# lmb-freiburg/locov

Hardware: AMD Instinct MI355X
Metric: proposals/sec through LSM ROI-head (1333x800, 1000 prop, 1203-class text bank) (higher is better)
Workload: dtype f32 (Res5 GEMM products formed from f16x2 split operands on the f16 matrix pipe, f32 accumulate; error vs f64 <= 1.5 x the f32-MFMA kernel's + 6e-7 and <= 3e-6 on every tested shape, tests/test_gpu_split_gemm.py)

## Files before the change

include/locov_hip.h:

```cpp
#ifndef LOCOV_HIP_H
#define LOCOV_HIP_H

#include <stdint.h>

#ifdef __cplusplus
extern "C" {
#endif

#define LOCOV_ABI_VERSION 8

#define LOCOV_OK 0
#define LOCOV_ERR_INVALID_ARG (-1)
#define LOCOV_ERR_LAUNCH (-2)
#define LOCOV_ERR_UNSUPPORTED (-3)

#define LOCOV_F32 0
#define LOCOV_BF16 1

#define LOCOV_NORM_NONE 0
#define LOCOV_NORM_L2 1
#define LOCOV_NORM_STANDARDIZE 2

#define LOCOV_EPI_RELU 1u
#define LOCOV_GEMM_A_SPLIT 0x1000u
// ... 428 lines not shown
} locov_weight_prep_job;
int locov_res5_weight_prep(const locov_weight_prep_job *jobs, int n_jobs, unsigned *overflow, locov_stream_t stream);

int locov_weight_transpose_scale(const float *w, int N, int K, const float *row_scale, float *out,
                                 locov_stream_t stream);
int locov_conv3x3_weight_flip(const float *w, int N, int Cin, const float *row_scale, float *out,
                              locov_stream_t stream);
int locov_im2col3x3_nhwc(const float *x, int64_t R, int H, int W, int C, float *col, locov_stream_t stream);
int locov_conv3x3_wgrad_unpack(const float *dw_packed, int N, int Cin, const float *row_scale, float *dw,
                               locov_stream_t stream);
int locov_relu_mask(const float *g, const float *act, int64_t n, float *out, float *amax_out, locov_stream_t stream);
#define LOCOV_ZERO_LIST_MAX 24
int locov_zero_if_raised(float *const *tensors, const int64_t *counts, int n_tensors, const unsigned *flag,
                         locov_stream_t stream);

int locov_spatial_mean_bwd(const float *g, const float *act, int64_t R, int C, int HW, float *out,
                           float *amax_out, locov_stream_t stream);
int locov_rows_stride2(const float *src, int N, int H, int W, int C, int forward, float *dst,
                       locov_stream_t stream);
int locov_roi_align_nhwc_bwd(const float *grad_rows, int64_t grad_ld, int N, int H, int W, int C,
                             const float *rois, int64_t R, int pooled_h, int pooled_w, float spatial_scale,
                             int sampling_ratio, int aligned, int bin_stride, int pos_major, float *grad_feat,
                             locov_stream_t stream);

#define LOCOV_REGIONS_MAX_B 64
#define LOCOV_REGIONS_MAX_CANDIDATES 4096
#define LOCOV_REGIONS_GRID 0
#define LOCOV_REGIONS_GRID_ALL 1
#define LOCOV_REGIONS_BOXES 2
#define LOCOV_REGIONS_ROWS 0
#define LOCOV_REGIONS_NCHW 1
int locov_regions_select(const double *keys, int mode, int B, const int *count_host, const int *ext_a_host,
                         const int *ext_b_host, int grid_w, const float *const *boxes_host, int n, int limit, int mask_w,
                         int mvm_w, int64_t *indices, int *src_row, int *inv, uint8_t *mask, float *loc, float *mvm,
                         locov_stream_t stream);
int locov_regions_gather_fwd(const float *src, int layout, int64_t ld, int B, int n, int C, int64_t hw, const int *src_row,
                             float *out, locov_stream_t stream);
int locov_regions_gather_bwd(const float *grad_out, int layout, int64_t ld, int64_t rows, int C, int64_t hw, const int *inv,
                             float *grad_src, locov_stream_t stream);

#define LOCOV_MHA_MAX_S 4096
#define LOCOV_MHA_MAX_GRID 65535
int locov_mha_fwd(const float *q, int64_t ldq, const float *k, int64_t ldk, const float *v, int64_t ldv, const float *bias,
                  const uint8_t *keep, float p_drop, float scale, int nseq, int S, int H, int d, float *ctx, int64_t ldo,
                  float *lse, locov_stream_t stream);
int locov_mha_bwd(const float *q, int64_t ldq, const float *k, int64_t ldk, const float *v, int64_t ldv, const float *bias,
// ... 68 lines not shown
```

locov_amd/_lib.py:

```python
from __future__ import annotations

import ctypes
import os
from ctypes import c_char_p, c_double, c_float,c_int, c_int64, c_uint, c_void_p, POINTER

HERE = os.path.dirname(os.path.abspath(__file__))
LIB_PATH = os.environ.get("LOCOV_HIP_LIB") or os.path.join(HERE, "liblocov_hip.so")

OK = 0
F32, BF16 = 0, 1
NORM_NONE, NORM_L2, NORM_STANDARDIZE = 0, 1, 2
EPI_RELU = 1
WINO_OUT_ROI_MAJOR = 0x100
WINO_IN_ROI_MAJOR = 0x200
SEGMEAN_RES_ROI_MAJOR = 0x400
GEMM_A_SPLIT = 0x1000
EPI_OUT_SPLIT = 0x2000
EPI_RES_SPLIT = 0x4000
MAX_LEVELS = 8
ZERO_LIST_MAX = 24
LABEL_MAX_IMAGES, LABEL_MAX_THRESHOLDS, SAMPLE_MAX_PROPOSALS = 64, 6, 4096
ABI_VERSION = 8
DETECT_MAX_CANDIDATES, DETECT_FLAG_NONFINITE, DETECT_FLAG_OVERFLOW = 8192, 1, 2
RPN_FLAG_NONFINITE, RPN_MAX_PRE_NMS_TOPK, RPN_MAX_ANCHORS = 1, 16384, (1 << 22) - 1
# ... 157 lines not shown
    "locov_winograd_wgrad_f32_split": (c_int, [_p, _p, c_int64, c_int, c_int, c_uint, _p, _p, _p, _p, c_int64, _p]),
    "locov_winograd_wgrad_f32_split_v": (c_int, [_p, _p, c_int64, c_int, c_int, c_uint, _p, _p, _p, _p, c_int64, _p]),
    "locov_conv1x1_winograd_workspace_bytes": (c_int64, [c_int64, c_int, c_int]),
    "locov_conv1x1_winograd_workspace_bytes_for": (c_int64, [c_int64, c_int, c_int, c_int, c_int64]),
    "locov_roi_align_winograd_workspace_bytes": (c_int64, [c_int64, c_int, c_int]),
    "locov_roi_align_winograd_conv3x3_f32_split": (c_int, [_p, c_int, c_int, c_int, c_int, c_int64, _p, c_int64, c_int, c_float, c_int, c_int,
                                                           _p, _p, _p, c_float, c_float, _p, _p, _p, c_int64, c_int, c_uint, c_float, _p, c_int64,
                                                           _p, _p]),
    "locov_conv1x1_winograd_conv3x3_f32_split": (c_int, [_p, c_int64, c_int, c_float, _p, c_float, _p, _p, c_int64, c_int, _p, c_float, c_float,
                                                         _p, _p, _p, c_int64, c_int, c_uint, c_float, _p, c_int64, _p, _p]),
    "locov_winograd_wgrad_workspace_bytes": (c_int64, [c_int64, c_int, c_int]),
    "locov_winograd_wgrad_f32": (c_int, [_p, _p, c_int64, c_int, c_int, c_uint, _p, _p, _p, c_int64, _p]),
    "locov_res5_weight_prep": (c_int, [POINTER(WeightPrepJob), c_int, _p, _p]),
    "locov_weight_transpose_scale": (c_int, [_p, c_int, c_int, _p, _p, _p]),
    "locov_conv3x3_weight_flip": (c_int, [_p, c_int, c_int, _p, _p, _p]),
    "locov_im2col3x3_nhwc": (c_int, [_p, c_int64, c_int, c_int, c_int, _p, _p]),
    "locov_conv3x3_wgrad_unpack": (c_int, [_p, c_int, c_int, _p, _p, _p]),
    "locov_relu_mask": (c_int, [_p, _p, c_int64, _p, _p, _p]),
    "locov_zero_if_raised": (c_int, [POINTER(c_void_p), POINTER(c_int64), c_int, _p, _p]),
    "locov_spatial_mean_bwd": (c_int, [_p, _p, c_int64, c_int, c_int, _p, _p, _p]),
    "locov_rows_stride2": (c_int, [_p, c_int, c_int, c_int, c_int, c_int, _p, _p]),
    "locov_roi_align_nhwc_bwd": (c_int, [_p, c_int64, c_int, c_int, c_int, c_int, _p, c_int64, c_int, c_int, c_float, c_int, c_int,
                                         c_int, c_int, _p, _p]),
    "locov_box_head_fwd": (c_int, [_p, c_int64, c_int, c_int, c_int, _p, _p, _p, _p, _p, _p, c_int, c_int,
                                   c_int, c_int, _p, _p, _p, _p, _p, _p]),
    "locov_regions_select": (c_int, [_p, c_int, c_int, POINTER(c_int), POINTER(c_int), POINTER(c_int), c_int, POINTER(c_void_p), c_int, c_int,
                                     c_int, c_int, _p, _p, _p, _p, _p, _p, _p]),
    "locov_regions_gather_fwd": (c_int, [_p, c_int, c_int64, c_int, c_int, c_int, c_int64, _p, _p, _p]),
    "locov_regions_gather_bwd": (c_int, [_p, c_int, c_int64, c_int64, c_int, c_int64, _p, _p, _p]),
    "locov_mha_fwd": (c_int, [_p, c_int64, _p, c_int64, _p, c_int64, _p, _p, c_float, c_float, c_int, c_int, c_int, c_int, _p, c_int64,
                              _p, _p]),
    "locov_mha_bwd": (c_int, [_p, c_int64, _p, c_int64, _p, c_int64, _p, _p, c_float, c_float, c_int, c_int, c_int, c_int, _p,
                              c_int64, _p, _p, _p, c_int64, _p, c_int64, _p, c_int64, _p]),
    "locov_resnet_stem_fwd": (c_int, [_p, c_int, c_int, c_int, _p, _p, _p, c_int, _p, _p]),
    "locov_resnet_stem_fwd_sel": (c_int, [_p, c_int, c_int, c_int, _p, _p, _p, c_int, _p, _p, _p]),
    "locov_resnet_stem_wgrad_workspace_bytes": (c_int64, [c_int, c_int, c_int]),
    "locov_resnet_stem_wgrad": (c_int, [_p, c_int, c_int, c_int, _p, _p, _p, c_int, _p, _p, c_int64, _p]),
    "locov_preprocess_images": (c_int, [POINTER(c_void_p), POINTER(c_int), POINTER(c_int), c_int, c_int, c_int, POINTER(c_float),
                                        POINTER(c_float), c_float, _p, c_int, c_int, _p]),
    "locov_detector_rescale": (c_int, [_p, POINTER(c_int), POINTER(c_float), POINTER(c_float), POINTER(c_int), POINTER(c_int), c_int,
                                       _p, _p, _p, _p]),
    "locov_caption_embed_fwd": (c_int, [_p, _p, c_int, c_int, c_int, c_int, _p, _p, c_int, _p, c_int, _p, _p, c_float, _p, c_float, c_double,
                                        c_double, c_double, c_int, c_int, c_int, _p, _p, _p, _p, _p, _p]),
    "locov_caption_embed_bwd_workspace_bytes": (c_int64, [c_int, c_int, c_int]),
    "locov_caption_embed_bwd": (c_int, [_p, c_int, c_int, c_int, c_int, _p, _p, _p, _p, _p, _p, _p, c_float, _p, _p, _p, _p, c_int64, _p]),
    "locov_sgd_workspace_bytes": (c_int64, [c_int, c_int64]),
# ... 43 lines not shown
```

locov_amd/csrc/roi_align_nhwc_bwd.hip:

```cpp
#include "roi_align_nhwc_common.h"

#include <cstdlib>

namespace locov {

__global__ __launch_bounds__(kNhwcThreads) void roi_align_nhwc_bwd_kernel(
    const float *__restrict__ grad_rows, int64_t grad_ld, float *__restrict__ grad_feat, int N, int H, int W, int C,
    const float *__restrict__ rois, int PH, int PW, float scale, int sampling_ratio, int aligned, int bin_stride, int OH, int OW,
    int pos_major, int nslices, int64_t R, int bwd_win_floats)
{
    extern __shared__ float bwd_win[];
    __shared__ AxisSampleN ytab[kMaxAxisN];
    __shared__ AxisSampleN xtab[kMaxAxisN];
    __shared__ float ypw[kSepCols * (kSepGrid + 1)];
    __shared__ float xpw[kSepCols * (kSepGrid + 1)];
    __shared__ int ypix[kSepCols][2];
    __shared__ int xpix[kSepCols][2];
    __shared__ int sep_bad;
    const NhwcRoiFrame f = nhwc_roi_frame(rois, N, H, W, C, PH, PW, scale, sampling_ratio, aligned, bin_stride, OH, OW, (int64_t)C,
                                          (unsigned)sizeof(float), nslices, R, NhwcRoiLds{ytab, xtab, ypw, xpw, ypix, xpix, &sep_bad});
    const float start_h = f.start_h, start_w = f.start_w, bin_h = f.bin_h, bin_w = f.bin_w, inv_count = f.inv_count;
    const int gh = f.gh, gw = f.gw, q_lo = f.q_lo;
    const unsigned xstride = f.xstride, ystride = f.ystride;
    const bool use_lds = f.use_lds, separable = f.separable, valid_b = f.valid_b;
// ... 94 lines not shown
            for (int ky = 0; ky < nyp; ky++)
                for (int kx = 0; kx < nxp; kx++) scatter(y0 + (unsigned)ky * ystride + (unsigned)kx * xstride, yw[ky] * xw[kx]);
        } else {
            for (int iy = 0; iy < gh; iy++) {
                const AxisSampleN ys = use_lds ? ytab[oh * gh + iy]
                                               : as_offsets(axis_sample_n(start_h, bin_h, oh * bin_stride, iy, gh, H), ystride);
                for (int ix = 0; ix < gw; ix++) {
                    const AxisSampleN xs = use_lds ? xtab[ow * gw + ix]
                                                   : as_offsets(axis_sample_n(start_w, bin_w, ow * bin_stride, ix, gw, W), xstride);
                    scatter((unsigned)ys.lo + (unsigned)xs.lo + ch_off, ys.wh * xs.wh);
                    scatter((unsigned)ys.lo + (unsigned)xs.hi + ch_off, ys.wh * xs.wl);
                    scatter((unsigned)ys.hi + (unsigned)xs.lo + ch_off, ys.wl * xs.wh);
                    scatter((unsigned)ys.hi + (unsigned)xs.hi + ch_off, ys.wl * xs.wl);
                }
            }
        }
        cq += kNhwcThreads;
        normalise();
    }
}

constexpr int kBT = 8, kBwdCh = 128, kBwdList = 2048;

__global__ __launch_bounds__(256, 3) void roi_align_even_bwd_tiles_kernel(const float *__restrict__ grad_rows, int64_t grad_ld,
                                                                      const float *__restrict__ rois, int R, int N, int H, int W, int C, int PH,
                                                                      int PW, float scale, int sampling_ratio, int aligned, int bin_stride,
                                                                      float *__restrict__ grad_feat, int nslices, int tiles_x, int tiles_y)
{
    constexpr int OB = 7;
    __shared__ float wy[4][OB][kBT];
    __shared__ float4 wx[4][OB];
    __shared__ unsigned short list[kBwdList];
    __shared__ int wave_cnt[4], list_n;
    const int tid = threadIdx.x, lane = tid & 63, wave = tid >> 6;
    int t = blockIdx.x;
    const int slice = t % nslices;
    t /= nslices;
    const int tx = t % tiles_x;
    t /= tiles_x;
    const int ty = t % tiles_y, img = t / tiles_y;
    const int ty0 = ty * kBT, tx0 = tx * kBT, c0 = slice * kBwdCh;
    float acc_r[kBT][kBT / 2];
#pragma unroll
    for (int py = 0; py < kBT; py++)
#pragma unroll
        for (int q = 0; q < kBT / 2; q++) acc_r[py][q] = 0.f;

    const int c = tid & (kBwdCh - 1), half = tid >> 7;

    for (int base = 0; base < R; base += kBwdList) {
        if (tid == 0) list_n = 0;
        __syncthreads();
        const int stop = min(R, base + kBwdList);
        for (int r0 = base; r0 < stop; r0 += 256) {
            const int r = r0 + tid;
            bool ok = false;
            if (r < stop) {
                const float *roi = rois + (int64_t)r * 5;
                if ((int)roi[0] == img) {
                    const RoiGeom g = roi_geom(roi, scale, PH, PW, sampling_ratio, aligned);
                    auto reaches = [](float a, float b, int t0) {
                        const float lo = a <= b ? a : b, hi = a <= b ? b : a;
                        return hi + 2.f >= (float)t0 && lo - 2.f <= (float)(t0 + kBT);
                    };
                    ok = reaches(g.start_h, g.start_h + g.bin_h * (float)PH, ty0) && reaches(g.start_w, g.start_w + g.bin_w * (float)PW, tx0) &&
                         g.grid_h > 0 && g.grid_w > 0;
                }
            }
            const unsigned long long b = __ballot(ok);
            if (lane == 0) wave_cnt[wave] = __popcll(b);
            __syncthreads();
// ... 22 lines not shown
                my = __ballot(w != 0.f);
                if (lane < OB * kBT) wyw[o][p] = w;
                w = 0.f;
                if (lane < OB * kBT)
                    for (int i = 0; i < g.grid_w; i++) {
                        const AxisSampleN sm = axis_sample_n(g.start_w, g.bin_w, o * bin_stride, i, g.grid_w, W);
                        w += (sm.lo == tx0 + p ? sm.wh : 0.f) + (sm.hi == tx0 + p ? sm.wl : 0.f);
                    }
                mx = __ballot(w != 0.f);
                if (lane < OB * kBT && (p & 1) == half) reinterpret_cast<float *>(&wxw[o])[p >> 1] = w;
            }
            __builtin_amdgcn_fence(__ATOMIC_RELEASE, "wavefront");
            __builtin_amdgcn_wave_barrier();
            __builtin_amdgcn_fence(__ATOMIC_ACQUIRE, "wavefront");
            if (my == 0 || mx == 0) continue;
            const float inv_count = 1.f / g.count;
            const float *grow = grad_rows + (int64_t)r * (OB * OB) * grad_ld + c0 + c;
            float gv[OB * OB];
#pragma unroll
            for (int oh = 0; oh < OB; oh++)
#pragma unroll
                for (int ow = 0; ow < OB; ow++)
                    gv[oh * OB + ow] = ((my >> (8 * oh)) & 0xffull) != 0 && ((mx >> (8 * ow)) & 0xffull) != 0 ? grow[(int64_t)(oh * OB + ow) * grad_ld] : 0.f;
#pragma unroll
            for (int oh = 0; oh < OB; oh++) {
                if (((my >> (8 * oh)) & 0xffull) == 0) continue;
                float tq[kBT / 2] = {0.f, 0.f, 0.f, 0.f};
#pragma unroll
                for (int ow = 0; ow < OB; ow++) {
                    const float4 w4 = wxw[ow];
                    const float gq = gv[oh * OB + ow];
                    tq[0] = fmaf(w4.x, gq, tq[0]);
                    tq[1] = fmaf(w4.y, gq, tq[1]);
                    tq[2] = fmaf(w4.z, gq, tq[2]);
                    tq[3] = fmaf(w4.w, gq, tq[3]);
                }
#pragma unroll
                for (int q = 0; q < kBT / 2; q++) tq[q] *= inv_count;
#pragma unroll
                for (int py = 0; py < kBT; py++) {
                    const float w = wyw[oh][py];
#pragma unroll
                    for (int q = 0; q < kBT / 2; q++) acc_r[py][q] = fmaf(w, tq[q], acc_r[py][q]);
                }
            }
            __builtin_amdgcn_fence(__ATOMIC_RELEASE, "wavefront");
            __builtin_amdgcn_wave_barrier();
        }
        __syncthreads();
    }
    __syncthreads();
#pragma unroll
    for (int py = 0; py < kBT; py++)
#pragma unroll
        for (int q = 0; q < kBT / 2; q++) {
            const int y = ty0 + py, x = tx0 + 2 * q + half;
            const float v = acc_r[py][q];
            if (y < H && x < W && v != 0.f) grad_feat[(((int64_t)img * H + y) * W + x) * C + c0 + c] += v;
        }
}

}

using namespace locov;

extern "C" {

int locov_roi_align_nhwc_bwd(const float *grad_rows, int64_t grad_ld, int N, int H, int W, int C, const float *rois, int64_t R,
                             int pooled_h, int pooled_w, float spatial_scale, int sampling_ratio, int aligned, int bin_stride,
                             int pos_major, float *grad_feat, locov_stream_t stream)
{
    LOCOV_REQUIRE(grad_ld >= C && grad_ld % 4 == 0, "locov_roi_align_nhwc_bwd: grad_ld must be >= C and a multiple of 4");
    LOCOV_REQUIRE((int64_t)H * W * C * 4 < 0xffffffffLL, "locov_roi_align_nhwc_bwd: one image must stay below 4 GiB");
    LOCOV_REQUIRE(R >= 0 && N > 0 && C > 0 && H > 0 && W > 0 && pooled_h > 0 && pooled_w > 0, "locov_roi_align_nhwc_bwd: bad shape");
    LOCOV_REQUIRE(spatial_scale > 0.f, "locov_roi_align_nhwc_bwd: spatial_scale must be > 0");
    LOCOV_REQUIRE(bin_stride == 1 || bin_stride == 2, "locov_roi_align_nhwc_bwd: bin_stride must be 1 or 2");
    LOCOV_REQUIRE(C % 4 == 0, "locov_roi_align_nhwc_bwd: C must be a multiple of 4");
    if (R == 0) return LOCOV_OK;
    LOCOV_REQUIRE(grad_rows && rois && grad_feat, "locov_roi_align_nhwc_bwd: null pointer");
    LOCOV_REQUIRE(R <= 0x7fffffffLL, "locov_roi_align_nhwc_bwd: R too large");
    LOCOV_REQUIRE(((uintptr_t)grad_rows | (uintptr_t)grad_feat) % 16 == 0, "locov_roi_align_nhwc_bwd: misaligned pointer");
    const int OH = (pooled_h + bin_stride - 1) / bin_stride, OW = (pooled_w + bin_stride - 1) / bin_stride;
    {
        const char *te = getenv("LOCOV_POOL_BWD_TILES");
        if ((!te || atoi(te) != 0) && OH == 7 && OW == 7 && !pos_major && C % kBwdCh == 0) {
            const int tiles_x = (W + kBT - 1) / kBT, tiles_y = (H + kBT - 1) / kBT, ns = C / kBwdCh;
            const int64_t wgs = (int64_t)N * tiles_x * tiles_y * ns;
            LOCOV_REQUIRE(wgs <= 0x7fffffffLL, "locov_roi_align_nhwc_bwd: map too large");
            hipLaunchKernelGGL(roi_align_even_bwd_tiles_kernel, dim3((unsigned)wgs), dim3(256), 0, as_stream(stream), grad_rows, grad_ld, rois, (int)R,
                               N, H, W, C, pooled_h, pooled_w, spatial_scale, sampling_ratio, aligned, bin_stride, grad_feat, ns, tiles_x, tiles_y);
            return check_launch("locov_roi_align_nhwc_bwd (tiles)");
        }
    }
    int nslices = nhwc_slices(C);
    while (nslices < 8 && C / (2 * nslices) >= 128 && (C >> 2) % (2 * nslices) == 0) nslices *= 2;
    LOCOV_REQUIRE(R * nslices <= 0x7fffffffLL, "locov_roi_align_nhwc_bwd: R too large");
    dim3 grid((unsigned)(R * nslices));
    const char *we = getenv("LOCOV_POOL_BWD_WINDOW");
    const int win_bytes = we ? atoi(we) : 20480;
    static std::atomic<int> window_lds[kMaxDevices];
    const bool attr_ok = raise_dynamic_lds(window_lds, reinterpret_cast<const void *>(&roi_align_nhwc_bwd_kernel), 65536, nullptr) == LOCOV_OK;
    const int wb = attr_ok && win_bytes > 0 ? (win_bytes < 65536 ? win_bytes : 65536) : 0;
    hipLaunchKernelGGL(roi_align_nhwc_bwd_kernel, grid, dim3(kNhwcThreads), (size_t)wb, as_stream(stream), grad_rows, grad_ld, grad_feat, N, H,
                       W, C, rois, pooled_h, pooled_w, spatial_scale, sampling_ratio, aligned, bin_stride, OH, OW, pos_major, nslices, R, wb / 4);
    return check_launch("locov_roi_align_nhwc_bwd");
}

}
```

locov_amd/ops.py:

```python
from __future__ import annotations

import ctypes
import itertools
import math
import threading
from typing import NamedTuple, Optional, Sequence, Tuple

import torch
from torch.autograd.function import once_differentiable

from . import _lib
from ._lib import BF16, F32, NORM_L2, NORM_NONE, NORM_STANDARDIZE, LocovError, check

__all__ = [
    "level_assign", "roi_align", "roi_align_levels", "nchw_to_nhwc", "roi_align_nhwc", "spatial_mean",
    "linear", "rownorm", "to_bf16", "sim_gemm_bf16", "box_head", "NORM_NONE", "NORM_L2",
    "NORM_STANDARDIZE", "F32", "BF16",
]


def _dev(t: torch.Tensor, name: str, dtype=torch.float32) -> torch.Tensor:
    if not isinstance(t, torch.Tensor):
        raise TypeError(f"{name} must be a torch.Tensor")
    if not t.is_cuda:
# ... 1330 lines not shown
    with torch.cuda.device(src.device):
        check(_lib.load().locov_rows_stride2(_ptr(src), N, H, W, C, int(forward), _ptr(out), _stream(src)), "locov_rows_stride2")
    return out


def roi_align_nhwc_bwd(grad_rows: torch.Tensor, feat_shape, rois: torch.Tensor, output_size: int, spatial_scale: float,
                       sampling_ratio: int = 0, aligned: bool = True, bin_stride: int = 1, pos_major: bool = False,
                       accumulate_into: Optional[torch.Tensor] = None) -> torch.Tensor:
    grad_rows = _rows(grad_rows, "grad_rows")
    rois = _dev(rois, "rois")
    N, H, W, C = feat_shape
    if accumulate_into is None:
        gf = torch.zeros((N, H, W, C), dtype=torch.float32, device=grad_rows.device)
    else:
        gf = _out(accumulate_into, (N, H, W, C), grad_rows, "roi_align_nhwc_bwd")
    with torch.cuda.device(gf.device):
        check(_lib.load().locov_roi_align_nhwc_bwd(_ptr(grad_rows), grad_rows.stride(0) if grad_rows.shape[0] else C, N, H, W, C,
                                                   _ptr(rois), rois.shape[0], output_size, output_size, float(spatial_scale),
                                                   int(sampling_ratio), int(aligned), int(bin_stride), int(pos_major), _ptr(gf),
                                                   _stream(gf)), "locov_roi_align_nhwc_bwd")
    return gf


def nhwc_to_nchw(x: torch.Tensor) -> torch.Tensor:
    x = _dev(x, "x")
    N, H, W, C = x.shape
    out = torch.empty((N, C, H, W), dtype=torch.float32, device=x.device)
    with torch.cuda.device(x.device):
        check(_lib.load().locov_nchw_to_nhwc(_ptr(x), N, H * W, C, 1, _ptr(out), F32, _stream(x)), "locov_nchw_to_nhwc")
    return out


def resnet_stem_shape(H: int, W: int) -> Tuple[int, int]:
    CH, CW = (H + 1) // 2, (W + 1) // 2
    return (CH + 1) // 2, (CW + 1) // 2


def resnet_stem(images: torch.Tensor, weight: torch.Tensor, scale: torch.Tensor, shift: torch.Tensor,
                out: Optional[torch.Tensor] = None) -> torch.Tensor:
    images, weight = _dev(images, "images"), _dev(weight, "weight")
    scale, shift = _dev(scale, "scale"), _dev(shift, "shift")
    if images.dim() != 4 or images.shape[1] != 3 or min(images.shape[2:]) < 1:
        raise ValueError(f"resnet_stem: images must be [N,3,H,W], got {tuple(images.shape)}")
    Cout = weight.shape[0]
    if tuple(weight.shape) != (Cout, 3, 7, 7) or tuple(scale.shape) != (Cout,) or tuple(shift.shape) != (Cout,):
        raise ValueError(f"resnet_stem: weight must be [Cout,3,7,7] and scale, shift [Cout], got {tuple(weight.shape)}, "
# ... 1285 lines not shown
```

locov_amd/res5_train.py:

```python
from __future__ import annotations

import os
from typing import List, NamedTuple, Optional, Sequence, Tuple

import torch

from . import ops

__all__ = ["res5_rows", "res5_grid", "res5_rois", "roi_align_even_rows", "to_nhwc", "Res5BlockFn", "Res5OutputFn", "Res5Step", "Segment",
           "saved_activations", "saved_activations_per_step"]

_BWD_STREAMS = bool(int(os.environ.get("LOCOV_RES5_BWD_STREAMS", "1")))
_SIDE_STREAMS = {}


def _side_stream(device) -> "torch.cuda.Stream":
    key = (torch.device(device), torch.cuda.current_stream(device).cuda_stream)
    st = _SIDE_STREAMS.get(key)
    if st is None:
        st = _SIDE_STREAMS[key] = torch.cuda.Stream(device=device)
    return st


_KEEP_V = bool(int(os.environ.get("LOCOV_RES5_KEEP_V", "1")))
_NO_WINO_BWD = bool(int(os.environ.get("LOCOV_RES5_BWD_DIRECT", "0")))
_BWD_F32 = bool(int(os.environ.get("LOCOV_RES5_BWD_F32", "0")))


def _wino_ok(H: int, W: int, cin: int, cout: int) -> bool:
    return H == 7 and W == 7 and cin % 32 == 0 and cout % 4 == 0


class Segment(NamedTuple):
    row0: int
    n: int
    H: int
    W: int

    @property
    def rows(self) -> int:
        return self.n * self.H * self.W

    @property
    def wino(self) -> bool:
        return self.H == 7 and self.W == 7


class Res5Step:

    def __init__(self, stage, split: bool, device, capacity_rows: int, grid: bool = True, rois: bool = True):
        self.stage, self.split, self.device = stage, bool(split), torch.device(device)
        self.operands = stage.train_operands(self.split, grid=grid, rois=rois)
        self.capacity = int(capacity_rows)
        self.segments: List[Segment] = []
        self.filled = 0
        self._pending: List[int] = []
        new = lambda c: torch.empty((self.capacity, c), dtype=torch.float32, device=self.device)
        self.x0 = new(stage[0].conv1.in_channels)
        self.act = [(new(b.conv1.out_channels), new(b.conv2.out_channels), new(b.conv3.out_channels)) for b in stage]
        self.cols = {}
        self.wino_ws = {}

    def input_rows(self, rows: int) -> torch.Tensor:
        row0 = self.filled + sum(self._pending)
        if row0 + rows > self.capacity:
            raise ValueError(f"Res5Step: {row0} + {rows} rows exceed the capacity of {self.capacity}")
        self._pending.append(rows)
        return self.x0[row0:row0 + rows]

    @torch.no_grad()
    def forward(self, n: int, H: int, W: int, on_range_final=None) -> Segment:
        return self.forward_segments([(n, H, W)], on_range_final)[0]

    @torch.no_grad()
    def forward_segments(self, geoms: Sequence[Tuple[int, int, int]], on_range_final=None) -> List[Segment]:
        assert [g[0] * g[1] * g[2] for g in geoms] == self._pending, "Res5Step.forward: input_rows() of every segment first"
        new = []
        for (n, H, W) in geoms:
            seg = Segment(self.filled, n, H, W)
            new.append((len(self.segments), seg))
            self.segments.append(seg)
            self.filled += seg.rows
        self._pending = []
        live = [(si, seg) for si, seg in new if seg.rows > 0]
        if not live:
            return [seg for _, seg in new]
        stage, T = self.stage, self.operands
        lo, hi = live[0][1].row0, live[-1][1].row0 + live[-1][1].rows
        joint = slice(lo, hi)
        x = self.x0[joint]
        nb = len(stage)
        for bi, blk in enumerate(stage):
            Y1, Y2, OUT = self.act[bi]
            s1, b1 = stage.operands.fold(blk.conv1)
            s2, b2 = stage.operands.fold(blk.conv2)
            s3, b3 = stage.operands.fold(blk.conv3)
            c2 = blk.conv2
            _linear(x, T.get(blk.conv1, "plain"), b1, scale=s1, relu=True, out=Y1[joint])
            if blk.shortcut is not None:
                ss, bs = stage.operands.fold(blk.shortcut)
                sc = _linear(x, T.get(blk.shortcut, "plain"), bs, scale=ss)
            else:
                sc = x
            last = bi == nb - 1
            w3 = T.get(blk.conv3, "plain")
            order = sorted(live, key=lambda it: self.seg_wino(it[1], c2)) if last else live
            for si, seg in order:
                sl = slice(seg.row0, seg.row0 + seg.rows)
                early = False
                if self.seg_wino(seg, c2):
                    u2 = T.get(c2, "wino")
                    early = (on_range_final is not None and last and blk.shortcut is None
                             and isinstance(u2, ops.SplitWeight) and isinstance(w3, ops.SplitWeight))
                    keep = None
                    if _KEEP_V and isinstance(u2, ops.SplitWeight) and c2.in_channels % 8 == 0 and seg.n > 0:
                        ws_bytes = ops.winograd_workspace_bytes(seg.n, c2.in_channels, c2.out_channels)
                        if ws_bytes == 121 * seg.n * (c2.in_channels + c2.out_channels) * 4 + 16:
                            keep = self.wino_ws[(bi, si)] = torch.empty(ws_bytes, dtype=torch.uint8, device=self.device)
                    ops.winograd_conv3x3(Y1[sl], u2, scale=s2, shift=b2, relu=True, roi_major=True, in_roi_major=True, out=Y2[sl],
                                         range_check_scale=16.0 if early else None, workspace=keep)
                    if early:
                        on_range_final()
                        on_range_final = None
                else:
                    col = self.cols[(bi, si)] = ops.im2col3x3(Y1[sl], seg.H, seg.W)
                    _linear(col, T.get(c2, "col"), b2, scale=s2, relu=True, out=Y2[sl])
                if last and len(live) > 1:
                    _linear(Y2[sl], w3, b3, scale=s3, residual=sc[sl.start - lo:sl.stop - lo], relu=True, out=OUT[sl])
            if not (last and len(live) > 1):
                _linear(Y2[joint], w3, b3, scale=s3, residual=sc, relu=True, out=OUT[joint])
            x = OUT[joint]
        return [seg for _, seg in new]

    def seg_wino(self, seg: Segment, c2) -> bool:
        return seg.wino and _wino_ok(seg.H, seg.W, c2.in_channels, c2.out_channels)

    def outputs(self, inputs: Sequence[torch.Tensor], pooled: Sequence[bool]) -> List[torch.Tensor]:
        assert len(inputs) == len(pooled) == len(self.segments) and not self._pending
        active = ops.active_guard(self.device) if self.split else None
        self.skip_words = [getattr(active, "step_word", active.word)] if active is not None and getattr(active, "deferred", False) else []
        self.bwd_split = self.split and not _BWD_F32
        self._carry = None
        self._prefetched = False
        self.need_x0 = any(t.requires_grad for t in inputs)
        h = None
        for bi, blk in enumerate(self.stage):
            head_w = (blk.conv1.weight,) + ((blk.shortcut.weight,) if blk.shortcut is not None else ())
            y1 = Res5BlockFn.apply(self, bi, "head", len(inputs), *inputs, *head_w) if bi == 0 else Res5BlockFn.apply(self, bi, "head", 1, h, *head_w)
            h = Res5BlockFn.apply(self, bi, "tail", 1, y1, blk.conv2.weight, blk.conv3.weight)
        outs = Res5OutputFn.apply(self, tuple(bool(p) for p in pooled), h)
        return list(outs) if isinstance(outs, tuple) else [outs]

    def _bwd_operands(self):
        sp = self.bwd_split
        return self.operands if self.operands.split == bool(sp) else self.stage.train_operands(bool(sp))

    def _bwd_guarded(self, fn):
        if not self.bwd_split:
# ... 237 lines not shown
    @staticmethod
    def _backward_head(ctx, g1):
        step, bi, n_in = ctx.step, ctx.bi, ctx.n_in
        stage, segs = step.stage, step.segments
        rows = step.filled
        blk = stage[bi]
        has_sc = blk.shortcut is not None
        first = bi == 0
        need_x = any(ctx.needs_input_grad[4:4 + n_in])
        need_w = ctx.needs_input_grad[4 + n_in:]
        gw: List[Optional[torch.Tensor]] = [None] * ctx.nw
        weights = (blk.conv1.weight,) + ((blk.shortcut.weight,) if has_sc else ())
        if rows == 0:
            step._carry = None
            if not first:
                gx = torch.empty((0, blk.conv1.in_channels), dtype=torch.float32, device=step.device)
                step._carry = ("tail", gx, None)
                return (gx,) + tuple(torch.zeros_like(w) if need else None for w, need in zip(weights, need_w))
            return tuple(None for _ in range(n_in)) + tuple(torch.zeros_like(w) if need else None for w, need in zip(weights, need_w))
        g1, sg1, g, sg = Res5BlockFn._take_carry(step, g1, "head")
        sp, T, slot, wgrad_1x1, dgrad_1x1 = Res5BlockFn._helpers(ctx)
        x, _ = ctx.saved_tensors
        s1 = stage.operands.fold(blk.conv1)[0]
        if need_w[0]:
            gw[0] = wgrad_1x1(g1, sg1, x, s1).view_as(blk.conv1.weight)
        if has_sc:
            ss = stage.operands.fold(blk.shortcut)[0]
            if need_w[1]:
                gw[1] = wgrad_1x1(g, sg, x, ss).view_as(blk.shortcut.weight)
        if not need_x:
            return tuple(None for _ in range(n_in)) + tuple(gw)
        mask = None if first else x
        gx, sgx = dgrad_1x1(g1, sg1, blk.conv1, amax_out=None if (first or has_sc) else slot(g1),
                            residual=None if has_sc else g, mask=None if has_sc else mask)
        if has_sc:
            gx, sgx = dgrad_1x1(g, sg, blk.shortcut, amax_out=None if first else slot(g), residual=gx, mask=mask)
        if not first:
            step._carry = ("tail", gx, sgx)
            return (gx,) + tuple(gw)
        gxs = [None] * n_in
        for i, seg in enumerate(segs):
            if ctx.needs_input_grad[4 + i]:
                gxs[i] = gx[seg.row0:seg.row0 + seg.rows]
        return tuple(gxs) + tuple(gw)


def saved_activations(out: torch.Tensor) -> List[torch.Tensor]:
    found, stack, seen = {}, [out.grad_fn], set()
    while stack:
        n = stack.pop()
        if n is None or id(n) in seen:
            continue
        seen.add(id(n))
        if "Res5BlockFn" in type(n).__name__:
            found[(n.bi, n.half)] = n
        stack += [f for f, _ in n.next_functions]
    saved = []
    for bi in sorted({k[0] for k in found}):
        x, y1 = found[(bi, "head")].saved_tensors
        _, y2, o = found[(bi, "tail")].saved_tensors
        saved += [x, y1, y2, o]
    return saved


def saved_activations_per_step(out: torch.Tensor) -> List[Tuple["Res5Step", List[torch.Tensor]]]:
    found, order, stack, seen = {}, [], [out.grad_fn], set()
# ... 101 lines not shown
    def forward(ctx, nhwc, step=None):
        N, H, W, _ = nhwc.shape
        ctx.dims = (N, H, W)
        dst = step.input_rows(N * ((H + 1) // 2) * ((W + 1) // 2)) if step is not None else None
        return ops.rows_stride2(nhwc.detach(), N, H, W, True, out=dst)

    @staticmethod
    def backward(ctx, g):
        N, H, W = ctx.dims
        return ops.rows_stride2(g, N, H, W, False), None


def grid_rows(nhwc: torch.Tensor, step=None) -> torch.Tensor:
    return _Stride2Rows.apply(nhwc, step)


def grid_segment(step: "Res5Step", nhwc: torch.Tensor) -> torch.Tensor:
    N, H, W, _ = nhwc.shape
    rows = grid_rows(nhwc, step)
    step.forward(N, (H + 1) // 2, (W + 1) // 2)
    return rows


def roi_segment(step: "Res5Step", nhwc: torch.Tensor, rois: torch.Tensor, P: int, scale: float, sampling_ratio: int, aligned: bool,
                on_range_final=None) -> torch.Tensor:
    x0 = roi_align_even_rows(nhwc, rois, P, scale, sampling_ratio, aligned, step)
    o = (int(P) + 1) // 2
    step.forward(rois.shape[0], o, o, on_range_final=on_range_final)
    return x0


def grid_and_roi_segments(step: "Res5Step", nhwc: torch.Tensor, rois: torch.Tensor, P: int, scale: float, sampling_ratio: int, aligned: bool,
                          on_range_final=None):
    N, H, W, _ = nhwc.shape
    rows = grid_rows(nhwc, step)
    x0 = roi_align_even_rows(nhwc, rois, P, scale, sampling_ratio, aligned, step)
    o = (int(P) + 1) // 2
    step.forward_segments([(N, (H + 1) // 2, (W + 1) // 2), (rois.shape[0], o, o)], on_range_final=on_range_final)
    return rows, x0


def grid_capacity(nhwc: torch.Tensor) -> int:
    N, H, W, _ = nhwc.shape
    return N * ((H + 1) // 2) * ((W + 1) // 2)


def to_nchw(rows: torch.Tensor, N: int, OH: int, OW: int, channels_last: bool = False) -> torch.Tensor:
    if channels_last:
        return rows.view(N, OH, OW, rows.shape[1]).permute(0, 3, 1, 2)
    return _ToNCHW.apply(rows.view(N, OH, OW, rows.shape[1]))


def res5_grid(stage, nhwc: torch.Tensor, split: bool = True, overflow_check: bool = True, on_overflow=None,
              channels_last: bool = False) -> torch.Tensor:
    N, H, W, _ = nhwc.shape
    assert stage.supports_rows_path() and stage[0].stride == 2 and stage[0].stride_in_1x1
    OH, OW = (H + 1) // 2, (W + 1) // 2
    made = {}

# ... 21 lines not shown
```

Baseline: 403,600.

## Run res5 block-0 1x1 convs on the feature map before ROI align

Block 0's conv1 and shortcut 1x1 convolutions are linear, so they commute with ROI-align bilinear sampling. When the pooled rows (49 per ROI) outnumber the map pixels by a set factor, the new path runs the GEMMs on the feature map and then ROI-aligns the products, applying the folded scale, shift and ReLU inside the align. Backward gets a new fused ROI-align kernel that scatters both gradient blocks into one map for the weight and input gradients. This trades GEMM work that scales with the ROI count for map-sized GEMMs, at the cost of more code paths and an env-controlled heuristic.

```diff
diff --git a/include/locov_hip.h b/include/locov_hip.h
--- a/include/locov_hip.h
+++ b/include/locov_hip.h
@@ -474,6 +474,12 @@
                              const float *rois, int64_t R, int pooled_h, int pooled_w, float spatial_scale,
                              int sampling_ratio, int aligned, int bin_stride, int pos_major, float *grad_feat,
                              locov_stream_t stream);
+int locov_roi_align_nhwc_affine_bwd(const float *grad0, int64_t grad0_ld, int C0, const float *scale0, const float *mask0,
+                                    int64_t mask0_ld, const float *grad1, int64_t grad1_ld, int C1, const float *scale1,
+                                    const float *mask1, int64_t mask1_ld, int N, int H, int W, const float *rois, int64_t R,
+                                    int pooled_h, int pooled_w, float spatial_scale, int sampling_ratio, int aligned,
+                                    int bin_stride, float *grad_feat, int64_t feat_ld, int accumulate, float *amax_out,
+                                    locov_stream_t stream);
 
 #define LOCOV_REGIONS_MAX_B 64
 #define LOCOV_REGIONS_MAX_CANDIDATES 4096
diff --git a/locov_amd/_lib.py b/locov_amd/_lib.py
--- a/locov_amd/_lib.py
+++ b/locov_amd/_lib.py
@@ -203,6 +203,9 @@
     "locov_rows_stride2": (c_int, [_p, c_int, c_int, c_int, c_int, c_int, _p, _p]),
     "locov_roi_align_nhwc_bwd": (c_int, [_p, c_int64, c_int, c_int, c_int, c_int, _p, c_int64, c_int, c_int, c_float, c_int, c_int,
                                          c_int, c_int, _p, _p]),
+    "locov_roi_align_nhwc_affine_bwd": (c_int, [_p, c_int64, c_int, _p, _p, c_int64, _p, c_int64, c_int, _p, _p, c_int64, c_int, c_int,
+                                                c_int, _p, c_int64, c_int, c_int, c_float, c_int, c_int, c_int, _p, c_int64, c_int, _p,
+                                                _p]),
     "locov_box_head_fwd": (c_int, [_p, c_int64, c_int, c_int, c_int, _p, _p, _p, _p, _p, _p, c_int, c_int,
                                    c_int, c_int, _p, _p, _p, _p, _p, _p]),
     "locov_regions_select": (c_int, [_p, c_int, c_int, POINTER(c_int), POINTER(c_int), POINTER(c_int), c_int, POINTER(c_void_p), c_int, c_int,
diff --git a/locov_amd/csrc/roi_align_nhwc_bwd.hip b/locov_amd/csrc/roi_align_nhwc_bwd.hip
--- a/locov_amd/csrc/roi_align_nhwc_bwd.hip
+++ b/locov_amd/csrc/roi_align_nhwc_bwd.hip
@@ -1,4 +1,5 @@
 #include "roi_align_nhwc_common.h"
+#include "gemm_nt.h"
 
 #include <cstdlib>
 
@@ -140,10 +141,27 @@
 
 constexpr int kBT = 8, kBwdCh = 128, kBwdList = 2048;
 
+struct BwdBlock {
+    const float *grad;
+    int64_t ld;
+    const float *scale;
+    const float *mask;
+    int64_t mask_ld;
+};
+struct BwdAffine {
+    BwdBlock blk[2];
+    int slices0;
+    int64_t out_ld;
+    int accumulate;
+    float *amax_out;
+};
+
+template <bool kAffine>
 __global__ __launch_bounds__(256, 3) void roi_align_even_bwd_tiles_kernel(const float *__restrict__ grad_rows, int64_t grad_ld,
                                                                       const float *__restrict__ rois, int R, int N, int H, int W, int C, int PH,
                                                                       int PW, float scale, int sampling_ratio, int aligned, int bin_stride,
-                                                                      float *__restrict__ grad_feat, int nslices, int tiles_x, int tiles_y)
+                                                                      float *__restrict__ grad_feat, int nslices, int tiles_x, int tiles_y,
+                                                                      BwdAffine ax)
 {
     constexpr int OB = 7;
     __shared__ float wy[4][OB][kBT];
@@ -165,6 +183,19 @@
         for (int q = 0; q < kBT / 2; q++) acc_r[py][q] = 0.f;
 
     const int c = tid & (kBwdCh - 1), half = tid >> 7;
+    float ch_scale = 1.f;
+    const float *mask_rows = nullptr;
+    int64_t mask_ld = 0;
+    if constexpr (kAffine) {
+        const bool second = slice >= ax.slices0;
+        const BwdBlock bk = second ? ax.blk[1] : ax.blk[0];
+        const int cb = (second ? slice - ax.slices0 : slice) * kBwdCh + c;
+        grad_rows = bk.grad + cb - (c0 + c);
+        grad_ld = bk.ld;
+        if (bk.scale != nullptr) ch_scale = bk.scale[cb];
+        if (bk.mask != nullptr) mask_rows = bk.mask + cb;
+        mask_ld = bk.mask_ld;
+    }
 
     for (int base = 0; base < R; base += kBwdList) {
         if (tid == 0) list_n = 0;
@@ -233,6 +264,20 @@
 #pragma unroll
                 for (int ow = 0; ow < OB; ow++)
                     gv[oh * OB + ow] = ((my >> (8 * oh)) & 0xffull) != 0 && ((mx >> (8 * ow)) & 0xffull) != 0 ? grow[(int64_t)(oh * OB + ow) * grad_ld] : 0.f;
+            if constexpr (kAffine) {
+#pragma unroll
+                for (int k = 0; k < OB * OB; k++) gv[k] *= ch_scale;
+                if (mask_rows != nullptr) {
+                    const float *mrow = mask_rows + (int64_t)r * (OB * OB) * mask_ld;
+#pragma unroll
+                    for (int oh = 0; oh < OB; oh++)
+#pragma unroll
+                        for (int ow = 0; ow < OB; ow++)
+                            if (((my >> (8 * oh)) & 0xffull) != 0 && ((mx >> (8 * ow)) & 0xffull) != 0 &&
+                                !(mrow[(int64_t)(oh * OB + ow) * mask_ld] > 0.f))
+                                gv[oh * OB + ow] = 0.f;
+                }
+            }
 #pragma unroll
             for (int oh = 0; oh < OB; oh++) {
                 if (((my >> (8 * oh)) & 0xffull) == 0) continue;
@@ -261,6 +306,24 @@
         __syncthreads();
     }
     __syncthreads();
+    if constexpr (kAffine) {
+        float m = 0.f;
+#pragma unroll
+        for (int py = 0; py < kBT; py++)
+#pragma unroll
+            for (int q = 0; q < kBT / 2; q++) {
+                const int y = ty0 + py, x = tx0 + 2 * q + half;
+                if (y < H && x < W) {
+                    float *p = grad_feat + (((int64_t)img * H + y) * W + x) * ax.out_ld + c0 + c;
+                    float v = acc_r[py][q];
+                    if (ax.accumulate) v = *p + v;
+                    *p = v;
+                    m = fmaxf(m, fabsf(v));
+                }
+            }
+        if (ax.amax_out != nullptr) amax_fold(ax.amax_out, m);
+        return;
+    }
 #pragma unroll
     for (int py = 0; py < kBT; py++)
 #pragma unroll
@@ -298,8 +361,9 @@
             const int tiles_x = (W + kBT - 1) / kBT, tiles_y = (H + kBT - 1) / kBT, ns = C / kBwdCh;
             const int64_t wgs = (int64_t)N * tiles_x * tiles_y * ns;
             LOCOV_REQUIRE(wgs <= 0x7fffffffLL, "locov_roi_align_nhwc_bwd: map too large");
-            hipLaunchKernelGGL(roi_align_even_bwd_tiles_kernel, dim3((unsigned)wgs), dim3(256), 0, as_stream(stream), grad_rows, grad_ld, rois, (int)R,
-                               N, H, W, C, pooled_h, pooled_w, spatial_scale, sampling_ratio, aligned, bin_stride, grad_feat, ns, tiles_x, tiles_y);
+            hipLaunchKernelGGL(roi_align_even_bwd_tiles_kernel<false>, dim3((unsigned)wgs), dim3(256), 0, as_stream(stream), grad_rows, grad_ld, rois,
+                               (int)R, N, H, W, C, pooled_h, pooled_w, spatial_scale, sampling_ratio, aligned, bin_stride, grad_feat, ns, tiles_x, tiles_y,
+                               BwdAffine{});
             return check_launch("locov_roi_align_nhwc_bwd (tiles)");
         }
     }
@@ -317,4 +381,35 @@
     return check_launch("locov_roi_align_nhwc_bwd");
 }
 
-}
+int locov_roi_align_nhwc_affine_bwd(const float *grad0, int64_t grad0_ld, int C0, const float *scale0, const float *mask0, int64_t mask0_ld,
+                                    const float *grad1, int64_t grad1_ld, int C1, const float *scale1, const float *mask1, int64_t mask1_ld,
+                                    int N, int H, int W, const float *rois, int64_t R, int pooled_h, int pooled_w, float spatial_scale,
+                                    int sampling_ratio, int aligned, int bin_stride, float *grad_feat, int64_t feat_ld, int accumulate,
+                                    float *amax_out, locov_stream_t stream)
+{
+    LOCOV_REQUIRE(bin_stride == 2 && pooled_h == 14 && pooled_w == 14, "locov_roi_align_nhwc_affine_bwd: only the even bins of a 14 x 14 pooler");
+    LOCOV_REQUIRE(C0 > 0 && C0 % kBwdCh == 0 && C1 >= 0 && C1 % kBwdCh == 0,
+                  "locov_roi_align_nhwc_affine_bwd: every column block must be a multiple of 128 channels");
+    LOCOV_REQUIRE(R >= 0 && R <= 0x7fffffffLL && N > 0 && H > 0 && W > 0, "locov_roi_align_nhwc_affine_bwd: bad shape");
+    LOCOV_REQUIRE(spatial_scale > 0.f, "locov_roi_align_nhwc_affine_bwd: spatial_scale must be > 0");
+    LOCOV_REQUIRE(feat_ld >= (int64_t)C0 + C1 && grad_feat != nullptr && (uintptr_t)grad_feat % 16 == 0 && feat_ld % 4 == 0,
+                  "locov_roi_align_nhwc_affine_bwd: grad_feat must be 16-byte aligned with a pixel pitch >= C0 + C1");
+    LOCOV_REQUIRE(R == 0 || rois != nullptr, "locov_roi_align_nhwc_affine_bwd: null rois");
+    const BwdBlock blocks[2] = {{grad0, grad0_ld, scale0, mask0, mask0_ld}, {grad1, grad1_ld, scale1, mask1, mask1_ld}};
+    const int cs[2] = {C0, C1};
+    for (int b = 0; b < 2; b++) {
+        if (cs[b] == 0 || R == 0) continue;
+        LOCOV_REQUIRE(blocks[b].grad != nullptr && blocks[b].ld >= cs[b], "locov_roi_align_nhwc_affine_bwd: gradient block null or its pitch below its width");
+        LOCOV_REQUIRE(blocks[b].mask == nullptr || blocks[b].mask_ld >= cs[b], "locov_roi_align_nhwc_affine_bwd: mask pitch below the block's width");
+    }
+    const int tiles_x = (W + kBT - 1) / kBT, tiles_y = (H + kBT - 1) / kBT, ns = (C0 + C1) / kBwdCh;
+    const int64_t wgs = (int64_t)N * tiles_x * tiles_y * ns;
+    LOCOV_REQUIRE(wgs <= 0x7fffffffLL, "locov_roi_align_nhwc_affine_bwd: map too large");
+    BwdAffine ax{{blocks[0], blocks[1]}, C0 / kBwdCh, feat_ld, accumulate != 0, amax_out};
+    hipLaunchKernelGGL(roi_align_even_bwd_tiles_kernel<true>, dim3((unsigned)wgs), dim3(256), 0, as_stream(stream), (const float *)nullptr, (int64_t)0,
+                       rois, (int)R, N, H, W, C0 + C1, pooled_h, pooled_w, spatial_scale, sampling_ratio, aligned, bin_stride, grad_feat, ns, tiles_x,
+                       tiles_y, ax);
+    return check_launch("locov_roi_align_nhwc_affine_bwd");
+}
+
+}
diff --git a/locov_amd/ops.py b/locov_amd/ops.py
--- a/locov_amd/ops.py
+++ b/locov_amd/ops.py
@@ -1376,6 +1376,45 @@
     return gf
 
 
+def roi_align_affine_bwd_ok(output_size: int, bin_stride: int, channels) -> bool:
+    return output_size == 14 and bin_stride == 2 and 1 <= len(channels) <= 2 and all(c > 0 and c % 128 == 0 for c in channels)
+
+
+def roi_align_nhwc_affine_bwd(blocks, feat_shape, rois: torch.Tensor, output_size: int, spatial_scale: float,
+                              sampling_ratio: int = 0, aligned: bool = True, bin_stride: int = 2,
+                              out: Optional[torch.Tensor] = None, accumulate: bool = False,
+                              amax_out: Optional[torch.Tensor] = None) -> torch.Tensor:
+    N, H, W = feat_shape
+    blocks = [(_rows(g, "grad_rows"), _dev(s, "ch_scale") if s is not None else None, _rows(m, "mask") if m is not None else None)
+              for g, s, m in blocks]
+    cs = [g.shape[1] for g, _, _ in blocks]
+    if not roi_align_affine_bwd_ok(output_size, bin_stride, cs):
+        raise ValueError("roi_align_nhwc_affine_bwd: the even bins of a 14 x 14 pooler, one or two blocks of multiples of 128 channels")
+    rois = _dev(rois, "rois")
+    R, C = rois.shape[0], sum(cs)
+    for g, s, m in blocks:
+        if g.shape[0] != 49 * R or (s is not None and s.numel() != g.shape[1]) or (m is not None and m.shape != g.shape):
+            raise ValueError("roi_align_nhwc_affine_bwd: a block's rows / scale / mask do not match")
+    if out is None:
+        if accumulate:
+            raise ValueError("roi_align_nhwc_affine_bwd: accumulate needs out")
+        out = torch.empty((N, H, W, C), dtype=torch.float32, device=rois.device)
+    ov = out.view(N * H * W, -1) if out.dim() == 4 and out.is_contiguous() else out
+    if (ov.dim() != 2 or ov.shape != (N * H * W, C) or ov.dtype != torch.float32 or not ov.is_cuda or ov.stride(1) != 1
+            or ov.stride(0) < C or ov.stride(0) % 4 or ov.data_ptr() % 16):
+        raise ValueError("roi_align_nhwc_affine_bwd: out must be the fp32 device map [N,H,W,C] or its pixel rows [N*H*W, C]")
+    args = []
+    for g, s, m in blocks + [(None, None, None)] * (2 - len(blocks)):
+        args += [_ptr(g), g.stride(0) if g is not None else 0, g.shape[1] if g is not None else 0, _ptr(s), _ptr(m),
+                 m.stride(0) if m is not None else 0]
+    with torch.cuda.device(rois.device):
+        check(_lib.load().locov_roi_align_nhwc_affine_bwd(*args, N, H, W, _ptr(rois), R, output_size, output_size, float(spatial_scale),
+                                                          int(sampling_ratio), int(aligned), int(bin_stride), _ptr(ov), ov.stride(0),
+                                                          int(accumulate), _ptr(amax_out), _stream(rois)),
+              "locov_roi_align_nhwc_affine_bwd")
+    return out
+
+
 def nhwc_to_nchw(x: torch.Tensor) -> torch.Tensor:
     x = _dev(x, "x")
     N, H, W, C = x.shape
diff --git a/locov_amd/res5_train.py b/locov_amd/res5_train.py
--- a/locov_amd/res5_train.py
+++ b/locov_amd/res5_train.py
@@ -29,6 +29,20 @@
 
 def _wino_ok(H: int, W: int, cin: int, cout: int) -> bool:
     return H == 7 and W == 7 and cin % 32 == 0 and cout % 4 == 0
+
+
+MAP_PAYS = 2.0
+
+
+def block0_on_map(stage, n_rois: int, n_pixels: int, P: int) -> bool:
+    mode = os.environ.get("LOCOV_TRAIN_BLOCK0", "auto")
+    if mode not in ("rows", "map", "auto"):
+        raise ValueError(f"LOCOV_TRAIN_BLOCK0={mode!r}: rows, map or auto")
+    b0 = stage[0]
+    if (mode == "rows" or b0.shortcut is None or n_rois <= 0 or b0.conv1.in_channels % 32
+            or not ops.roi_align_affine_bwd_ok(int(P), 2, [b0.conv1.out_channels, b0.shortcut.out_channels])):
+        return False
+    return mode == "map" or 49 * n_rois >= MAP_PAYS * n_pixels
 
 
 class Segment(NamedTuple):
@@ -60,6 +74,16 @@
         self.act = [(new(b.conv1.out_channels), new(b.conv2.out_channels), new(b.conv3.out_channels)) for b in stage]
         self.cols = {}
         self.wino_ws = {}
+        self.map_head = None
+        self._map_pending = None
+        self.map_si = None
+
+    def map_rows(self, nhwc: torch.Tensor, rois: torch.Tensor, P: int, scale: float, sampling_ratio: int, aligned: bool) -> None:
+        assert self.map_head is None, "Res5Step: one segment on the map"
+        self.map_head = (ops._dev(nhwc.detach(), "nhwc"), ops._dev(rois, "rois"), (int(P), float(scale), int(sampling_ratio), bool(aligned)))
+        self._map_pending = len(self._pending)
+        o = (int(P) + 1) // 2
+        self.input_rows(o * o * rois.shape[0])
 
     def input_rows(self, rows: int) -> torch.Tensor:
         row0 = self.filled + sum(self._pending)
@@ -76,8 +100,10 @@
     def forward_segments(self, geoms: Sequence[Tuple[int, int, int]], on_range_final=None) -> List[Segment]:
         assert [g[0] * g[1] * g[2] for g in geoms] == self._pending, "Res5Step.forward: input_rows() of every segment first"
         new = []
-        for (n, H, W) in geoms:
+        for j, (n, H, W) in enumerate(geoms):
             seg = Segment(self.filled, n, H, W)
+            if j == self._map_pending:
+                self.map_si, self._map_pending = len(self.segments), None
             new.append((len(self.segments), seg))
             self.segments.append(seg)
             self.filled += seg.rows
@@ -96,12 +122,15 @@
             s2, b2 = stage.operands.fold(blk.conv2)
             s3, b3 = stage.operands.fold(blk.conv3)
             c2 = blk.conv2
-            _linear(x, T.get(blk.conv1, "plain"), b1, scale=s1, relu=True, out=Y1[joint])
-            if blk.shortcut is not None:
-                ss, bs = stage.operands.fold(blk.shortcut)
-                sc = _linear(x, T.get(blk.shortcut, "plain"), bs, scale=ss)
+            if bi == 0 and any(si == self.map_si for si, _ in live):
+                sc = self._head_on_map(live, lo, hi)
             else:
-                sc = x
+                _linear(x, T.get(blk.conv1, "plain"), b1, scale=s1, relu=True, out=Y1[joint])
+                if blk.shortcut is not None:
+                    ss, bs = stage.operands.fold(blk.shortcut)
+                    sc = _linear(x, T.get(blk.shortcut, "plain"), bs, scale=ss)
+                else:
+                    sc = x
             last = bi == nb - 1
             w3 = T.get(blk.conv3, "plain")
             order = sorted(live, key=lambda it: self.seg_wino(it[1], c2)) if last else live
@@ -134,6 +163,30 @@
 
     def seg_wino(self, seg: Segment, c2) -> bool:
         return seg.wino and _wino_ok(seg.H, seg.W, c2.in_channels, c2.out_channels)
+
+    def _head_on_map(self, live, lo: int, hi: int) -> torch.Tensor:
+        b0, T = self.stage[0], self.operands
+        fold = self.stage.operands.fold
+        (s1, b1), (ss, bs) = fold(b0.conv1), fold(b0.shortcut)
+        w1, ws = T.get(b0.conv1, "plain"), T.get(b0.shortcut, "plain")
+        Y1 = self.act[0][0]
+        nhwc, rois, (P, scale, sampling_ratio, aligned) = self.map_head
+        N, H, W, cin = nhwc.shape
+        sc = torch.empty((hi - lo, b0.shortcut.out_channels), dtype=torch.float32, device=self.device)
+        for si, seg in live:
+            sl = slice(seg.row0, seg.row0 + seg.rows)
+            rel = slice(seg.row0 - lo, seg.row0 - lo + seg.rows)
+            if si != self.map_si:
+                _linear(self.x0[sl], w1, b1, scale=s1, relu=True, out=Y1[sl])
+                _linear(self.x0[sl], ws, bs, scale=ss, out=sc[rel])
+                continue
+            xm = nhwc.view(N * H * W, cin)
+            m1 = _linear(xm, w1).view(N, H, W, -1)
+            ops.roi_align_nhwc(m1, rois, P, scale, sampling_ratio, aligned, bin_stride=2, out=Y1[sl], ch_scale=s1, ch_shift=b1, relu=True)
+            del m1
+            ms = _linear(xm, ws).view(N, H, W, -1)
+            ops.roi_align_nhwc(ms, rois, P, scale, sampling_ratio, aligned, bin_stride=2, out=sc[rel], ch_scale=ss, ch_shift=bs)
+        return sc
 
     def outputs(self, inputs: Sequence[torch.Tensor], pooled: Sequence[bool]) -> List[torch.Tensor]:
         assert len(inputs) == len(pooled) == len(self.segments) and not self._pending
@@ -417,6 +470,8 @@
         sp, T, slot, wgrad_1x1, dgrad_1x1 = Res5BlockFn._helpers(ctx)
         x, _ = ctx.saved_tensors
         s1 = stage.operands.fold(blk.conv1)[0]
+        if first and step.map_si is not None and segs[step.map_si].rows > 0:
+            return Res5BlockFn._backward_head_on_map(ctx, x, g1, sg1, g, sg)
         if need_w[0]:
             gw[0] = wgrad_1x1(g1, sg1, x, s1).view_as(blk.conv1.weight)
         if has_sc:
@@ -437,6 +492,47 @@
         for i, seg in enumerate(segs):
             if ctx.needs_input_grad[4 + i]:
                 gxs[i] = gx[seg.row0:seg.row0 + seg.rows]
+        return tuple(gxs) + tuple(gw)
+
+
+    @staticmethod
+    def _backward_head_on_map(ctx, x, g1, sg1, g, sg):
+        step, n_in = ctx.step, ctx.n_in
+        blk, segs = step.stage[0], step.segments
+        need_in = ctx.needs_input_grad[4:4 + n_in]
+        need_w = ctx.needs_input_grad[4 + n_in:]
+        sp, T, slot, wgrad_1x1, dgrad_1x1 = Res5BlockFn._helpers(ctx)
+        fold = step.stage.operands.fold
+        s1, ss = fold(blk.conv1)[0], fold(blk.shortcut)[0]
+        nhwc, rois, (P, scale, sampling_ratio, aligned) = step.map_head
+        N, H, W, cin = nhwc.shape
+        mid = g1.shape[1]
+        mseg = segs[step.map_si]
+        msl = slice(mseg.row0, mseg.row0 + mseg.rows)
+        dmap = torch.empty((N * H * W, mid + g.shape[1]), dtype=torch.float32, device=step.device)
+        sm = slot(dmap)
+        ops.roi_align_nhwc_affine_bwd([(g1[msl], None, None), (g[msl], None, None)], (N, H, W), rois, P, scale, sampling_ratio, aligned,
+                                      bin_stride=2, out=dmap, amax_out=sm)
+        xm = nhwc.view(N * H * W, cin)
+        parts = [(dmap[:, :mid], dmap[:, mid:], sm, sm, xm, need_in[step.map_si])]
+        for i, seg in enumerate(segs):
+            if i != step.map_si and seg.rows > 0:
+                sl = slice(seg.row0, seg.row0 + seg.rows)
+                parts.append((g1[sl], g[sl], sg1, sg, x[sl], need_in[i]))
+        gw: List[Optional[torch.Tensor]] = [None, None]
+        for wi, (conv, s_) in enumerate(((blk.conv1, s1), (blk.shortcut, ss))):
+            if need_w[wi]:
+                for p in parts:
+                    part = wgrad_1x1(p[wi], p[2 + wi], p[4], s_)
+                    gw[wi] = part if gw[wi] is None else gw[wi].add_(part)
+                gw[wi] = gw[wi].view_as(conv.weight)
+        gxs: List[Optional[torch.Tensor]] = [None] * n_in
+        order = [step.map_si] + [i for i, seg in enumerate(segs) if i != step.map_si and seg.rows > 0]
+        for i, p in zip(order, parts):
+            if p[5]:
+                gx, _ = dgrad_1x1(p[0], p[2], blk.conv1)
+                gx, _ = dgrad_1x1(p[1], p[3], blk.shortcut, residual=gx)
+                gxs[i] = gx.view(N, H, W, cin) if i == step.map_si else gx
         return tuple(gxs) + tuple(gw)
 
 
@@ -584,9 +680,17 @@
     return rows
 
 
+def _roi_input(step: "Res5Step", nhwc: torch.Tensor, rois: torch.Tensor, P, scale, sampling_ratio, aligned) -> torch.Tensor:
+    N, H, W, _ = nhwc.shape
+    if nhwc.is_contiguous() and block0_on_map(step.stage, rois.shape[0], N * H * W, P):
+        step.map_rows(nhwc, rois, P, scale, sampling_ratio, aligned)
+        return nhwc
+    return roi_align_even_rows(nhwc, rois, P, scale, sampling_ratio, aligned, step)
+
+
 def roi_segment(step: "Res5Step", nhwc: torch.Tensor, rois: torch.Tensor, P: int, scale: float, sampling_ratio: int, aligned: bool,
                 on_range_final=None) -> torch.Tensor:
-    x0 = roi_align_even_rows(nhwc, rois, P, scale, sampling_ratio, aligned, step)
+    x0 = _roi_input(step, nhwc, rois, P, scale, sampling_ratio, aligned)
     o = (int(P) + 1) // 2
     step.forward(rois.shape[0], o, o, on_range_final=on_range_final)
     return x0
@@ -596,7 +700,7 @@
                           on_range_final=None):
     N, H, W, _ = nhwc.shape
     rows = grid_rows(nhwc, step)
-    x0 = roi_align_even_rows(nhwc, rois, P, scale, sampling_ratio, aligned, step)
+    x0 = _roi_input(step, nhwc, rois, P, scale, sampling_ratio, aligned)
     o = (int(P) + 1) // 2
     step.forward_segments([(N, (H + 1) // 2, (W + 1) // 2), (rois.shape[0], o, o)], on_range_final=on_range_final)
     return rows, x0
```

Measured after the change: 403,000. Within noise of the previous version (-0.1%).
